# AlexandreGac/alphazero-chess

Measured on AMD Instinct MI355X. Metric: MCTS sims/sec at 800 sims/move, 20x256 net; self-play games/hr at 1/2/4/8 GPU, higher is better.
Workload: dtype f32

## Files before the change

alphazero-chess_amd/azchess/_lib.py:

```python
import ctypes as C
import os

import numpy as np

_HERE = os.path.dirname(os.path.abspath(__file__))
LIB_PATH = os.environ.get("AZ_LIB") or os.path.join(_HERE, "libaz.so")
CSRC = os.path.join(os.path.dirname(_HERE), "csrc")

ACTION_SPACE = 4096
MAX_MOVES = 256
ONGOING, DRAW, WHITE_WINS, BLACK_WINS, ILLEGAL = 0, 1, 2, 3, -1
DTYPE_F32, DTYPE_BF16, DTYPE_FP8 = 0, 1, 2
EVAL_NET, EVAL_SYNTHETIC, EVAL_CALLBACK = 0, 1, 2
PACKED_KINDS = ("conv_w", "conv_b", "in_pk32", "wino_w", "wino16_w", "wino16_us", "w8", "w8s", "b8", "head",
                "head_frag", "head_frag32")


class AzPos(C.Structure):
    _fields_ = [("bb", C.c_uint64 * 8), ("turn", C.c_uint8), ("castling", C.c_uint8), ("ep", C.c_uint8),
                ("flags", C.c_uint8), ("halfmoves", C.c_uint16), ("fullmoves", C.c_uint16),
                ("rep_key", C.c_uint64)]


POS_DTYPE = np.dtype({
# ... 67 lines not shown
    ("az_pos_encode", C.c_int, [P(AzPos), P(C.c_float)]),
    ("az_game_create", C.c_int, [P(C.c_void_p)]),
    ("az_game_clone", C.c_int, [C.c_void_p, P(C.c_void_p)]),
    ("az_game_destroy", C.c_int, [C.c_void_p]),
    ("az_game_position", C.c_int, [C.c_void_p, P(AzPos)]),
    ("az_game_history", C.c_int, [C.c_void_p, P(C.c_int32), C.c_int]),
    ("az_game_play", C.c_int, [C.c_void_p, C.c_int32]),
    ("az_net_num_params", C.c_size_t, [C.c_int, C.c_int]),
    ("az_net_create", C.c_int, [P(AzNetDesc), P(C.c_float), C.c_size_t, C.c_int, P(C.c_void_p)]),
    ("az_net_destroy", C.c_int, [C.c_void_p]),
    ("az_net_tower_kernel", C.c_int, [C.c_void_p, C.c_char_p, C.c_int]),
    ("az_net_wino_streamed_points", C.c_int, [C.c_void_p]),
    ("az_net_wino_accumulators", C.c_int, [C.c_void_p]),
    ("az_net_wino_v_rows", C.c_int, [C.c_void_p]),
    ("az_wino_vrows_layout", C.c_int, [C.c_void_p] * 5),
    ("az_wino16_pack", C.c_int, [P(C.c_float), C.c_int, C.c_int, P(C.c_uint16), C.c_size_t, P(C.c_float)]),
    ("az_wino16_pack_rows", C.c_int, [P(C.c_float), C.c_int, P(C.c_uint16), C.c_size_t, P(C.c_float)]),
    ("az_net_load_mpk",C.c_int, [C.c_char_p, C.c_int, C.c_int, P(C.c_float), C.c_size_t]),
    ("az_net_save_mpk", C.c_int, [C.c_char_p, C.c_int, C.c_int, P(C.c_float), C.c_size_t]),
    ("az_net_forward", C.c_int, [C.c_void_p, P(C.c_float), C.c_int, P(C.c_float), P(C.c_float)]),
    ("az_net_forward_device", C.c_int, [C.c_void_p, C.c_void_p, C.c_int, C.c_void_p, C.c_void_p, C.c_void_p]),
    ("az_net_update_device", C.c_int, [C.c_void_p, C.c_void_p, C.c_size_t, C.c_void_p]),
    ("az_net_update", C.c_int, [C.c_void_p, P(C.c_float), C.c_size_t]),
    ("az_net_update_from_trainer", C.c_int, [C.c_void_p, C.c_void_p]),
    ("az_net_generation", C.c_int64, [C.c_void_p]),
    ("az_net_get_weights", C.c_int, [C.c_void_p, P(C.c_float), C.c_size_t]),
    ("az_net_packed_read", C.c_int, [C.c_void_p, C.c_int, C.c_int, C.c_void_p, C.c_size_t]),
    ("az_search_default_cfg", C.c_int, [P(AzSearchCfg)]),
    ("az_search_create", C.c_int, [C.c_void_p, P(AzSearchCfg), C.c_int, P(C.c_void_p)]),
    ("az_search_destroy", C.c_int, [C.c_void_p]),
# ... 127 lines not shown
```

alphazero-chess_amd/azchess/agent.py:

```python
import ctypes as C
import os

import numpy as np

from . import _lib as L
from .parameters import NUM_FILTERS, NUM_RES_BLOCKS, SEED


def num_params(blocks, filters):
    return int(L.lib.az_net_num_params(int(blocks), int(filters)))


def param_shapes(blocks, filters):
    F = filters
    out = [("input_conv.weight", (F, 19, 3, 3), 19 * 9), ("input_conv.bias", (F,), 19 * 9),
           ("input_bn", (4, F), None)]
    for b in range(blocks):
        for k in (1, 2):
            out += [("res_blocks.%d.conv%d.weight" % (b, k), (F, F, 3, 3), F * 9),
                    ("res_blocks.%d.conv%d.bias" % (b, k), (F,), F * 9),
                    ("res_blocks.%d.bn%d" % (b, k), (4, F), None)]
    out += [("policy_conv_1.weight", (32, F, 1, 1), F), ("policy_conv_1.bias", (32,), F), ("policy_bn", (4, 32), None),
            ("policy_conv_2.weight", (64, 32, 1, 1), 32), ("policy_conv_2.bias", (64,), 32),
            ("value_conv.weight", (8, F, 1, 1), F), ("value_conv.bias", (8,), F), ("value_bn", (4, 8), None),
# ... 95 lines not shown
        return buf.value.decode()

    @property
    def wino_streamed_points(self):
        return L.check(L.lib.az_net_wino_streamed_points(self._h))

    @property
    def wino_accumulators(self):
        return L.check(L.lib.az_net_wino_accumulators(self._h))

    @property
    def wino_v_rows(self):
        return L.check(L.lib.az_net_wino_v_rows(self._h))

    @property
    def winograd(self):
        return "Winograd" in self.tower_kernel

    def __del__(self):
        try:
            L.lib.az_net_destroy(self._h)
        except Exception:
            pass

    def save_file(self, path):
        save_mpk(path, self.weights, self.blocks, self.filters)

    def forward(self, x):
        x = np.ascontiguousarray(x, np.float32).reshape(-1, 19 * 64)
        n = x.shape[0]
        pol = np.zeros((n, 4096), np.float32)
        val = np.zeros(n, np.float32)
        L.check(L.lib.az_net_forward(self._h, L.fptr(x), n, L.fptr(pol), L.fptr(val)))
        return pol, val


def wino_vrows_layout():
    t = dict(write=np.empty((16, 64, 4), np.int32), read=np.empty((2, 4, 4, 64), np.int32),
             act=np.empty((16, 64, 4), np.int32), item=np.empty((2, 8, 4), np.int32), dims=np.empty(4, np.int32))
    L.check(L.lib.az_wino_vrows_layout(*(t[k].ctypes.data_as(C.c_void_p) for k in ("write", "read", "act", "item", "dims"))))
    return t


def mx8_quantize(x):
    x = np.ascontiguousarray(x, np.float32)
    if x.size % 32:
        raise ValueError("mx8_quantize: %d values are not whole blocks of 32" % x.size)
    codes = np.empty(x.shape, np.uint8)
    scales = np.empty(x.size // 32, np.uint8)
    u8 = lambda a: a.ctypes.data_as(L.P(C.c_uint8))
    L.check(L.lib.az_mx8_quantize(L.fptr(x), x.size // 32, u8(codes), u8(scales)))
    return codes, scales


def mx8_conv_probe(filters, act_codes, act_scales, w_codes, w_scales, bias, residual=None, device=0):
# ... 21 lines not shown
```

alphazero-chess_amd/csrc/api.hip:

```cpp
#include <string.h>

#include <cstdio>
#include <string>
#include <vector>

#include "az_internal.h"

namespace azi {
static thread_local std::string g_err;
void set_error(const std::string& m) { g_err = m; }
int fail(const std::string& m) { g_err = m; return -1; }
}

using namespace azi;

namespace {
inline const azc::Pos& P(const az_pos* p) { return *reinterpret_cast<const azc::Pos*>(p); }
inline azc::Pos& P(az_pos* p) { return *reinterpret_cast<azc::Pos*>(p); }

struct VecSink {
    int32_t* out; int cap; int n;
    void operator()(int idx) {
        const int reps = (idx & azc::PROMO_FLAG) ? 4 : 1;
        for (int r = 0; r < reps; r++) { if (n < cap) out[n] = idx & azc::IDX_MASK; n++; }
// ... 256 lines not shown
    return n->fused && tower_supported(n) && wino_split16(n) ? n->wino_streamed : 0;
}

int az_net_wino_accumulators(az_net* net) {
    if (!net) return fail("null argument");
    const NetDev* n = net->dev;
    return n->fused && tower_supported(n) && wino_split16(n) ? (n->wino_rows ? 8 : 16) : 0;
}

int az_net_wino_v_rows(az_net* net) {
    if (!net) return fail("null argument");
    const NetDev* n = net->dev;
    return n->fused && tower_supported(n) && wino_split16(n) && n->wino_rows && n->wino_vrows ? 1 : 0;
}

int az_wino16_pack(const float* folded, int filters, int streamed, uint16_t* out, size_t cap, float* unscale) {
    return wino16_pack(folded, filters, streamed, out, cap, unscale);
}

int az_wino16_pack_rows(const float* folded, int filters, uint16_t* out, size_t cap, float* unscale) {
    return wino16_pack_rows(folded, filters, out, cap, unscale);
}

static int ensure_scratch(NetDev* n, int rows) {
    if (rows <= n->scratch_rows) return 0;
    (void)hipFree(n->x); (void)hipFree(n->h); (void)hipFree(n->planes);
    n->x = n->h = n->planes = nullptr;
    const size_t ab = act_bytes(n->dtype);
    AZ_HIP(hipMalloc(&n->x, (size_t)rows * 64 * n->filters * ab));
    AZ_HIP(hipMalloc(&n->h, (size_t)rows * 64 * n->filters * ab));
// ... 46 lines not shown
```

alphazero-chess_amd/csrc/az_internal.h:

```cpp
#pragma once
#include <hip/hip_runtime.h>
#include <stdint.h>
#include <string>
#include <vector>

#include "../../include/az.h"
#include "chess.h"

static_assert(sizeof(az_pos) == 80, "az_pos layout");
static_assert(sizeof(azc::Pos) == sizeof(az_pos), "Pos == az_pos");

#ifndef AZ_WINOGRAD_DEFAULT
#define AZ_WINOGRAD_DEFAULT 1
#endif
#ifndef AZ_WINO_SPLIT16_DEFAULT
#define AZ_WINO_SPLIT16_DEFAULT 1
#endif
#ifndef AZ_WINO_DERIVE_DEFAULT
#define AZ_WINO_DERIVE_DEFAULT 1
#endif
#ifndef AZ_WINO_ROWS_DEFAULT
#define AZ_WINO_ROWS_DEFAULT 1
#endif
#ifndef AZ_WINO_VROWS_DEFAULT
#define AZ_WINO_VROWS_DEFAULT 1
#endif
#ifndef AZ_WINO_VROWS_SCHED
#define AZ_WINO_VROWS_SCHED 0
#endif
#ifndef AZ_WINO_ROWS_PF
#define AZ_WINO_ROWS_PF 4
#endif

namespace azi {

constexpr float WINO16_SA = 64.0f;
static inline bool wino16_selected(int level, int filters) {
    return filters == 256 ? level >= 1 : (filters == 128 || filters == 64) && level >= 2;
}

static inline int wino16_streamed(bool derive, int filters) { return derive && filters == 256 ? 12 : 16; }
constexpr int WINO_ROWS_PF = AZ_WINO_ROWS_PF;
static_assert(12 % WINO_ROWS_PF == 0 && WINO_ROWS_PF >= 2, "the ring's slots must be compile-time");
static inline bool wino16_rows(bool derive, bool rows, int filters) { return wino16_streamed(derive, filters) == 12 && rows; }
static inline bool wino16_vrows(bool rows_form, bool vrows) { return rows_form && vrows; }

void set_error(const std::string& msg);
int fail(const std::string& msg);

#define AZ_HIP(expr)                                                                        \
    do {                                                                                    \
        hipError_t e_ = (expr);                                                             \
        if (e_ != hipSuccess)                                                               \
            return ::azi::fail(std::string(#expr) + ": " + hipGetErrorString(e_));          \
    } while (0)

__device__ __forceinline__ int load_fresh(const int* p) {
    return __hip_atomic_load(p, __ATOMIC_RELAXED, __HIP_MEMORY_SCOPE_AGENT);
}
__device__ __forceinline__ int vgpr_index(int i) {
// ... 87 lines not shown
    std::vector<float*> conv_b;
    std::vector<size_t> conv_bytes;
    std::vector<void*> wino_w;
    std::vector<size_t> wino_bytes;
    bool winograd = AZ_WINOGRAD_DEFAULT != 0;
    std::vector<void*> wino16_w;
    std::vector<size_t> wino16_bytes;
    std::vector<float> wino16_us;
    int split16 = AZ_WINO_SPLIT16_DEFAULT;
    bool wino_derive = AZ_WINO_DERIVE_DEFAULT != 0;
    int wino_streamed = 16;
    bool wino_rows_env = AZ_WINO_ROWS_DEFAULT != 0;
    bool wino_rows = false;
    bool wino_vrows_env = AZ_WINO_VROWS_DEFAULT != 0;
    bool wino_vrows = false;
    float* head = nullptr;
    void* head_frag = nullptr;
    void* in_pk32 = nullptr;
    size_t in_pk32_bytes = 0;
    void* head_frag32 = nullptr;
    void* w8 = nullptr; void* w8s = nullptr; float* b8 = nullptr;
    size_t w8_bytes = 0, w8s_bytes = 0;
    size_t head_floats = 0;
    hipStream_t stream = nullptr;
    bool fused = true;
    void* x = nullptr; void* h = nullptr; void* planes = nullptr; int scratch_rows = 0;
    float* d_in = nullptr; float* d_pol = nullptr; float* d_val = nullptr; int io_rows = 0;
    int64_t generation = 0;
    struct NetUpdate* upd = nullptr;
};
// ... 61 lines not shown
```

alphazero-chess_amd/csrc/net.hip:

```cpp
#include <math.h>
#include <string.h>

#include <algorithm>
#include <cstdio>
#include <cstdlib>

#include "az_internal.h"

namespace azi {

typedef __attribute__((ext_vector_type(8))) __bf16 bf16x8;
typedef __attribute__((ext_vector_type(4))) float f32x4;
typedef __attribute__((ext_vector_type(4))) __bf16 bf16x4;

template <typename T> struct DTraits;
template <> struct DTraits<__bf16> { static constexpr int CH_SLOT = 8; static constexpr int CHUNK = 32; };
template <> struct DTraits<float> { static constexpr int CH_SLOT = 4; static constexpr int CHUNK = 16; };

template <typename T> __device__ __forceinline__ float to_f(T v) { return (float)v; }

size_t act_bytes(int dtype) { return dtype == AZ_DTYPE_F32 ? 4 : 2; }

double net_tower_flop_per_eval(int B, int F) {
    return 2.0 * 64.0 * (171.0 * F + 18.0 * B * (double)F * F);
// ... 521 lines not shown
    const bool fp8 = d->dtype == AZ_DTYPE_FP8;
    if (fp8 && F != 128 && F != 256) return fail("AZ_DTYPE_FP8: the MX-fp8 tower supports 128 or 256 filters, not " + std::to_string(F));
    if (fp8 && B > 40) return fail("AZ_DTYPE_FP8: at most 40 blocks");
    if (fp8 && getenv("AZ_FUSED_TOWER") && atoi(getenv("AZ_FUSED_TOWER")) == 0)
        return fail("AZ_DTYPE_FP8 has only the fused tower kernel (AZ_FUSED_TOWER=0 is set)");
    if (n != az_net_num_params(B, F)) return fail("weight count mismatch");
    AZ_HIP(hipSetDevice(device));
    NetDev* net = new NetDev();
    net->blocks = B; net->filters = F; net->dtype = d->dtype; net->device = device;
    if (const char* e = getenv("AZ_FUSED_TOWER")) net->fused = atoi(e) != 0;
    if (const char* e = getenv("AZ_WINOGRAD")) net->winograd = atoi(e) != 0;
    if (const char* e = getenv("AZ_WINO_SPLIT16")) net->split16 = atoi(e);
    if (const char* e = getenv("AZ_WINO_DERIVE")) net->wino_derive = atoi(e) != 0;
    if (const char* e = getenv("AZ_WINO_ROWS")) net->wino_rows_env = atoi(e) != 0;
    if (const char* e = getenv("AZ_WINO_VROWS")) net->wino_vrows_env = atoi(e) != 0;
    AZ_HIP(hipStreamCreateWithFlags(&net->stream, hipStreamNonBlocking));
    const float* p = wts;
    std::vector<uint8_t> w8h, w8sh;
    std::vector<float> b8h;
    auto fold_conv = [&](int cin, const float* w, const float* bias, const float* bn) {
        const float *gamma = bn, *beta = bn + F, *mean = bn + 2 * F, *var = bn + 3 * F;
        std::vector<float> wf((size_t)F * cin * 9);
        std::vector<float> bf(F);
        for (int co = 0; co < F; co++) {
            const double sc = (double)gamma[co] / sqrt((double)var[co] + 1e-5);
            for (int k = 0; k < cin * 9; k++) wf[(size_t)co * cin * 9 + k] = (float)(w[(size_t)co * cin * 9 + k] * sc);
            bf[co] = (float)(((double)bias[co] - mean[co]) * sc + beta[co]);
        }
        if (fp8 && cin == F) {
            mx8_append_conv(wf, F, &w8h, &w8sh);
// ... 24 lines not shown
        }
        const bool h16 = d->dtype == AZ_DTYPE_F32 && cin == F && net->winograd && wino16_selected(net->split16, F);
        if (d->dtype == AZ_DTYPE_F32 && F >= 64 && cin == F && !h16) {
            auto u = winograd_f32(wf, F);
            void* du = nullptr;
            if (hipMalloc(&du, u.size() * 4) != hipSuccess) return -1;
            if (hipMemcpy(du, u.data(), u.size() * 4, hipMemcpyHostToDevice) != hipSuccess) return -1;
            net->wino_w.push_back(du);
            net->wino_bytes.push_back(u.size() * 4);
        }
        if (h16) {
            float us = 1.0f;
            net->wino_streamed = wino16_streamed(net->wino_derive, F);
            net->wino_rows = wino16_rows(net->wino_derive, net->wino_rows_env, F);
            net->wino_vrows = wino16_vrows(net->wino_rows, net->wino_vrows_env);
            auto u = net->wino_rows ? winograd_split16_rows(wf.data(), F, &us)
                                    : winograd_split16(wf.data(), F, net->wino_streamed, &us);
            void* du = nullptr;
            if (hipMalloc(&du, u.size() * 2) != hipSuccess) return -1;
            if (hipMemcpy(du, u.data(), u.size() * 2, hipMemcpyHostToDevice) != hipSuccess) return -1;
            net->wino16_w.push_back(du);
            net->wino16_bytes.push_back(u.size() * 2);
            net->wino16_us.push_back(us);
        }
        if (hipMalloc(&db, F * 4) != hipSuccess) return -1;
        if (hipMemcpy(db, bf.data(), F * 4, hipMemcpyHostToDevice) != hipSuccess) return -1;
        net->conv_w.push_back(dw);
        net->conv_b.push_back(db);
        return 0;
    };
// ... 81 lines not shown
}

void net_destroy(NetDev* n) {
    if (!n) return;
    (void)hipSetDevice(n->device);
    for (void* w : n->conv_w) (void)hipFree(w);
    for (void* w : n->wino_w) (void)hipFree(w);
    for (void* w : n->wino16_w) (void)hipFree(w);
    for (float* b : n->conv_b) (void)hipFree(b);
    (void)hipFree(n->head);
    (void)hipFree(n->head_frag);
    (void)hipFree(n->head_frag32);
    (void)hipFree(n->in_pk32);
    (void)hipFree(n->w8); (void)hipFree(n->w8s); (void)hipFree(n->b8);
    (void)hipFree(n->x); (void)hipFree(n->h); (void)hipFree(n->planes);
    (void)hipFree(n->d_in); (void)hipFree(n->d_pol); (void)hipFree(n->d_val);
    net_update_free(n);
    if (n->stream) (void)hipStreamDestroy(n->stream);
    delete n;
}

int net_tower(NetDev* n, const void* planes, const int* count, int rows, void* x, void* h, hipStream_t st,
              hipEvent_t ev0, hipEvent_t ev1) {
    if (rows <= 0) return 0;
    const int F = n->filters;
    const bool bf = n->dtype == AZ_DTYPE_BF16;
    int rc = bf ? launch_conv<__bf16>(F, 32, false, planes, x, n->conv_w[0], n->conv_b[0], count, rows, st)
                : launch_conv<float>(F, 32, false, planes, x, n->conv_w[0], n->conv_b[0], count, rows, st);
    if (rc) return rc;
    for (int b = 0; b < n->blocks; b++) {
// ... 96 lines not shown
```

alphazero-chess_amd/csrc/tower.hip:

```cpp
#include <math.h>
#include <stdio.h>
#include <stdlib.h>
#include <string.h>

#include "az_internal.h"
#include "search_dev.h"
#include "wino.h"

#include "tower_dev.h"

namespace azi {

template <int F, bool SEARCH>
__device__ __forceinline__ void tower_board(const __bf16* __restrict__ planes, const TowerArgs& ta, int row0, int nb,
                                            float* __restrict__ pol_out, float* __restrict__ val_out,
                                            const SearchOut& so, int tid) {
    constexpr int BPB = TowerCfg<F>::BPB, WB = TowerCfg<F>::WB, BPW = BPB / WB, NCO = TowerCfg<F>::NCO;
    constexpr int NCW = F / (16 * NCO);
    constexpr int NT = NCW * WB * 64;
    constexpr int RSF = F / 8 + 2, RSI = 32 / 8 + 2;
    constexpr int XSZ = BPB * 64 * RSF;
    constexpr int ZN = 16 + F / 8;
    constexpr int HSZ0 = (HeadsScratch<HeadsCfg<F>::NB, NT>::FLOATS * 4 + 15) / 16;
    constexpr int HSZ = ((XSZ > HSZ0 ? XSZ : HSZ0) + 15) / 16 * 16;
// ... 505 lines not shown
    }
    heads_group<F, RSF, 1, NT, SEARCH, true, H16>(ldsb, reinterpret_cast<float*>(V), 0, 1, row0, tid, ta.head_frag32, ta.head,
                                             pol_out, val_out, so, tr);
    wino_stamp(tr, 3 + 64 * 20);
}

template <int F, bool SEARCH, bool H16, int SP = 16, bool ROWS = false, bool VROWS = false>
__global__ void __launch_bounds__(WinoCfg<F>::NWV * 64)
tower32w_kernel(const float* __restrict__ planes, TowerArgs ta, const int* __restrict__ count_ptr, int rows,
                float* __restrict__ pol_out, float* __restrict__ val_out, SearchOut so) {
    const int count = count_ptr ? min(load_fresh(count_ptr), rows) : rows;
    if ((int)blockIdx.x >= count) return;
    tower32w_board<F, SEARCH, H16, SP, ROWS, VROWS>(planes, ta, blockIdx.x, pol_out, val_out, so, threadIdx.x);
}

template <int F, bool BF16> struct SimsCfg { static constexpr int NT = WinoCfg<F>::NWV * 64; };
template <int F> struct SimsCfg<F, true> {
    static_assert(TowerCfg<F>::BPB == 1, "persistent bf16 kernel: one board per workgroup");
    static constexpr int NT = (F / (16 * TowerCfg<F>::NCO)) * TowerCfg<F>::WB * 64;
};
template <int F, bool BF16, bool H16 = false, int SP = 16, bool ROWS = false, bool VROWS = false>
__global__ void __launch_bounds__((SimsCfg<F, BF16>::NT))
k_sims32w(Engine E, TowerArgs ta, SearchOut so, int step0, int step1) {
    __shared__ int s_kind;
    if (!E.active[vgpr_index(blockIdx.x)]) return;
    for (int step = step0; step <= step1; step++) {
        const int tid = vgpr_index(threadIdx.x), g = vgpr_index(blockIdx.x);
        const int lane = tid & 63, w = __builtin_amdgcn_readfirstlane(tid >> 6);
        unsigned long long* tr = tt_slot(w);
        wino_stamp(tr, 1910);
// ... 93 lines not shown
    if (n->filters == FF) {                                                                            \
        k_sims32w<FF, false, H16, SP, ROWS, VR><<<E.G, SimsCfg<FF, false>::NT, 0, st>>>(E, ta, so, step0, step1); \
        return hipGetLastError() == hipSuccess ? 0 : fail("persistent simulation kernel launch failed"); \
    }
    if (wino_split16(n)) {
        if (n->wino_streamed == 12 && n->wino_rows && n->wino_vrows) { AZ_SIMS32W(256, true, 12, true, true) }
        if (n->wino_streamed == 12 && n->wino_rows) { AZ_SIMS32W(256, true, 12, true, false) }
        if (n->wino_streamed == 12) { AZ_SIMS32W(256, true, 12, false, false) }
        AZ_SIMS32W(256, true, 16, false, false) AZ_SIMS32W(128, true, 16, false, false) AZ_SIMS32W(64, true, 16, false, false)
    }
    AZ_SIMS32W(256, false, 16, false, false) AZ_SIMS32W(128, false, 16, false, false) AZ_SIMS32W(64, false, 16, false, false)
#undef AZ_SIMS32W
    return fail("persistent simulation kernel: unsupported filters");
}

int tower_forward(NetDev* n, const void* planes, const int* count, int rows, float* pol, float* val,
                  const SearchOut* so, hipStream_t st) {
    if (rows <= 0) return 0;
    if (!tower_supported(n)) return fail("fused tower: unsupported net");
    if (!planes && (!so || !so->npos)) return fail("fused tower: no planes and no leaf positions to encode");
    if (n->dtype == AZ_DTYPE_FP8) return tower8_forward(n, planes, count, rows, pol, val, so, st);
    TowerArgs ta = tower_args(n);
    SearchOut dummy;
    memset(&dummy, 0, sizeof(dummy));
    const SearchOut& s = so ? *so : dummy;
#define AZ_TOWER(FF)                                                                                           \
    if (n->filters == FF) {                                                                                    \
        constexpr int BPB = TowerCfg<FF>::BPB;                                                                 \
        constexpr int NT = (FF / (16 * TowerCfg<FF>::NCO)) * TowerCfg<FF>::WB * 64;                            \
        const int grid = (rows + BPB - 1) / BPB;                                                               \
// ... 7 lines not shown
        constexpr int NT = (FF / (16 * Tower32Cfg<FF>::NCO)) * Tower32Cfg<FF>::WB * 64;                        \
        const int grid = (rows + BPB - 1) / BPB;                                                               \
        if (so) tower32_kernel<FF, true><<<grid, NT, 0, st>>>((const float*)planes, ta, count, rows, pol, val, s); \
        else tower32_kernel<FF, false><<<grid, NT, 0, st>>>((const float*)planes, ta, count, rows, pol, val, s);  \
        return hipGetLastError() == hipSuccess ? 0 : fail("f32 tower launch failed");                          \
    }
    if (n->dtype == AZ_DTYPE_F32) {
#define AZ_TOWER32W(FF, H16, SP, ROWS, VR)                                                                       \
        if (n->filters == FF) {                                                                                \
            constexpr int NT = WinoCfg<FF>::NWV * 64;                                                          \
            if (so) tower32w_kernel<FF, true, H16, SP, ROWS, VR><<<rows, NT, 0, st>>>((const float*)planes, ta, count, rows, pol, val, s); \
            else tower32w_kernel<FF, false, H16, SP, ROWS, VR><<<rows, NT, 0, st>>>((const float*)planes, ta, count, rows, pol, val, s);  \
            return hipGetLastError() == hipSuccess ? 0 : fail("f32 Winograd tower launch failed");             \
        }
        if (wino_split16(n)) {
            if (n->wino_streamed == 12 && n->wino_rows && n->wino_vrows) { AZ_TOWER32W(256, true, 12, true, true) }
            if (n->wino_streamed == 12 && n->wino_rows) { AZ_TOWER32W(256, true, 12, true, false) }
            if (n->wino_streamed == 12) { AZ_TOWER32W(256, true, 12, false, false) }
            AZ_TOWER32W(256, true, 16, false, false) AZ_TOWER32W(128, true, 16, false, false) AZ_TOWER32W(64, true, 16, false, false)
        }
        if (wino_supported(n)) {
            AZ_TOWER32W(256, false, 16, false, false) AZ_TOWER32W(128, false, 16, false, false) AZ_TOWER32W(64, false, 16, false, false)
        }
#undef AZ_TOWER32W
        AZ_TOWER32(256) AZ_TOWER32(128) AZ_TOWER32(64) AZ_TOWER32(32)
        return fail("fused tower: unsupported filters");
    }
    AZ_TOWER(256) AZ_TOWER(128) AZ_TOWER(64) AZ_TOWER(32)
#undef AZ_TOWER
#undef AZ_TOWER32
// ... 15 lines not shown
        for (int b = 0; b < 4; b++)
            for (int lane = 0; lane < 64; lane++) {
                read[(i * 4 + b) * 64 + lane] = wino_vr_read(i, b, lane);
                read[((4 + i) * 4 + b) * 64 + lane] = wino_vr_lo(wino_vr_rlane(lane, i >> 1)) + wino_vr_rimm(i, b);
            }
    for (int sched = 0; sched < 2; sched++)
        for (int wave = 0; wave < 8; wave++)
            for (int it = 0; it < 4; it++) {
                const int nw = sched ? 8 : 4;
                item[(sched * 8 + wave) * 4 + it] = wave < nw && it < WINO_VR_ITEMS / nw ? wino_vr_item(wave, it, nw) : -1;
            }
    dims[0] = WINO_VR_PLANE; dims[1] = WINO_VR_BYTES; dims[2] = WINO_VR_R16; dims[3] = 4;
    return 0;
}

#ifdef AZ_TOWER_TRACE
extern "C" int az_tower_trace_read(unsigned long long* out, size_t n) {
    const size_t cap = sizeof(azi::az_tower_trace_buf) / sizeof(unsigned long long);
    if (hipDeviceSynchronize() != hipSuccess) return -1;
    return hipMemcpyFromSymbol(out, HIP_SYMBOL(azi::az_tower_trace_buf), (n < cap ? n : cap) * 8) == hipSuccess ? 0 : -1;
}
#endif
```

alphazero-chess_amd/csrc/wino.h:

```cpp
#pragma once
#include "az_internal.h"

namespace azi {

typedef __attribute__((ext_vector_type(4))) float f32x4;
typedef __attribute__((ext_vector_type(2))) float f32x2;

#define AZ_PK2(name, mods)                                                                    \
    __device__ __forceinline__ f32x2 name(f32x2 a, f32x2 b) {                                 \
        f32x2 r;                                                                              \
        asm("v_pk_add_f32 %0, %1, %2 " mods : "=v"(r) : "v"(a), "v"(b));                      \
        return r;                                                                             \
    }
#define AZ_PK3(name, mods)                                                                    \
    __device__ __forceinline__ f32x2 name(f32x2 a, f32x2 m, f32x2 b) {                        \
        f32x2 r;                                                                              \
        asm("v_pk_fma_f32 %0, %1, %2, %3 " mods : "=v"(r) : "v"(a), "v"(m), "v"(b));          \
        return r;                                                                             \
    }
AZ_PK2(pk_add, "")
AZ_PK2(pk_sub, "neg_lo:[0,1] neg_hi:[0,1]")
AZ_PK2(pk_rowa, "op_sel_hi:[1,0] neg_lo:[0,1]")
AZ_PK2(pk_rowb, "op_sel:[1,0] neg_lo:[0,1] neg_hi:[0,1]")
AZ_PK2(pk_negx_add, "neg_lo:[1,1]")
// ... 716 lines not shown
                    s1[j] = pk_sub(pk_sub(m[4 + j], m[8 + j]), m[12 + j]);
                }
            }
            const f32x2 q0 = pkc_fma(pk_add(pk_add(s0[0], s0[1]), s0[2]), us, br);
            const f32x2 q1 = pkc_fma(pk_sub(pk_sub(s0[1], s0[2]), s0[3]), us, br);
            const f32x2 q2 = pkc_fma(pk_add(pk_add(s1[0], s1[1]), s1[2]), us, br);
            const f32x2 q3 = pkc_fma(pk_sub(pk_sub(s1[1], s1[2]), s1[3]), us, br);
            y[n][0][2 * p] = q0.x; y[n][0][2 * p + 1] = q0.y;
            y[n][1][2 * p] = q1.x; y[n][1][2 * p + 1] = q1.y;
            y[n][2][2 * p] = q2.x; y[n][2][2 * p + 1] = q2.y;
            y[n][3][2 * p] = q3.x; y[n][3][2 * p + 1] = q3.y;
        }
    }
}

}
```

include/az.h:

```cpp
#ifndef AZ_H
#define AZ_H
#include <stddef.h>
#include <stdint.h>

#ifdef __cplusplus
extern "C" {
#endif

#define AZ_ACTION_SPACE 4096
#define AZ_PLANES 19
#define AZ_MAX_MOVES 256

enum { AZ_ONGOING = 0, AZ_DRAW = 1, AZ_WHITE_WINS = 2, AZ_BLACK_WINS = 3, AZ_ILLEGAL = -1 };

typedef struct az_pos {
    uint64_t bb[8];
    uint8_t turn, castling, ep, flags;
    uint16_t halfmoves, fullmoves;
    uint64_t rep_key;
} az_pos;

const char* az_last_error(void);
int az_version(void);
int az_device_count(int* n);
// ... 15 lines not shown
int az_game_destroy(az_game* g);
int az_game_position(const az_game* g, az_pos* out);
int az_game_history(const az_game* g, int32_t* moves, int cap);
int az_game_play(az_game* g, int32_t index);

enum { AZ_DTYPE_F32 = 0, AZ_DTYPE_BF16 = 1, AZ_DTYPE_FP8 = 2 };
typedef struct { int blocks, filters, dtype; } az_net_desc;
typedef struct az_net az_net;
size_t az_net_num_params(int blocks, int filters);
int az_net_create(const az_net_desc* desc, const float* weights, size_t n, int device, az_net** out);
int az_net_destroy(az_net* net);
int az_net_tower_kernel(az_net* net, char* out, int cap);
int az_net_wino_streamed_points(az_net* net);
int az_net_wino_accumulators(az_net* net);
int az_net_wino_v_rows(az_net* net);
int az_wino_vrows_layout(int* write, int* read, int* act, int* item, int* dims);
int az_net_load_mpk(const char* path, int blocks, int filters, float* out, size_t n);
int az_net_save_mpk(const char* path, int blocks, int filters, const float* w, size_t n);
int az_net_forward(az_net* net, const float* planes, int n, float* policy, float* value);
int az_net_forward_device(az_net* net, const float* d_planes, int n, float* d_policy, float* d_value,
                          void* stream);
int az_net_update_device(az_net* net, const float* d_weights, size_t n, void* stream);
int az_net_update(az_net* net, const float* weights, size_t n);
int64_t az_net_generation(az_net* net);
int az_net_get_weights(az_net* net, float* out, size_t n);
enum {
    AZ_PACKED_CONV_W = 0, AZ_PACKED_CONV_B = 1, AZ_PACKED_IN_PK32 = 2, AZ_PACKED_WINO_W = 3, AZ_PACKED_WINO16_W = 4,
    AZ_PACKED_WINO16_US = 5, AZ_PACKED_W8 = 6, AZ_PACKED_W8S = 7, AZ_PACKED_B8 = 8, AZ_PACKED_HEAD = 9,
    AZ_PACKED_HEAD_FRAG = 10, AZ_PACKED_HEAD_FRAG32 = 11, AZ_PACKED_KINDS = 12
};
// ... 167 lines not shown
```

Measured before the change: 191,600.

## Add two-board-per-workgroup Winograd tower kernel with global activation buffers

Adds a new fused tower kernel where each 512-thread workgroup runs two boards through the 20-block Winograd tower. Every weight fragment loaded from memory then feeds MFMAs for both boards, which halves weight traffic per board. Activations move from LDS to a per-stream global scratch buffer, leaving LDS room for two boards' transformed tiles. Waves coordinate through an LDS flag. It is on by default for 256-filter f32 split16 rows/vrows nets. The cost is extra global-memory round-trips for activations and more register pressure.

```diff
diff --git a/alphazero-chess_amd/azchess/_lib.py b/alphazero-chess_amd/azchess/_lib.py
--- a/alphazero-chess_amd/azchess/_lib.py
+++ b/alphazero-chess_amd/azchess/_lib.py
@@ -105,6 +105,8 @@
     ("az_net_wino_accumulators", C.c_int, [C.c_void_p]),
     ("az_net_wino_v_rows", C.c_int, [C.c_void_p]),
     ("az_wino_vrows_layout", C.c_int, [C.c_void_p] * 5),
+    ("az_net_wino_boards", C.c_int, [C.c_void_p]),
+    ("az_wino_boards_layout", C.c_int, [C.c_void_p] * 6),
     ("az_wino16_pack", C.c_int, [P(C.c_float), C.c_int, C.c_int, P(C.c_uint16), C.c_size_t, P(C.c_float)]),
     ("az_wino16_pack_rows", C.c_int, [P(C.c_float), C.c_int, P(C.c_uint16), C.c_size_t, P(C.c_float)]),
     ("az_net_load_mpk",C.c_int, [C.c_char_p, C.c_int, C.c_int, P(C.c_float), C.c_size_t]),
diff --git a/alphazero-chess_amd/azchess/agent.py b/alphazero-chess_amd/azchess/agent.py
--- a/alphazero-chess_amd/azchess/agent.py
+++ b/alphazero-chess_amd/azchess/agent.py
@@ -133,6 +133,10 @@
         return L.check(L.lib.az_net_wino_v_rows(self._h))
 
     @property
+    def wino_boards(self):
+        return L.check(L.lib.az_net_wino_boards(self._h))
+
+    @property
     def winograd(self):
         return "Winograd" in self.tower_kernel
 
@@ -158,6 +162,13 @@
     t = dict(write=np.empty((16, 64, 4), np.int32), read=np.empty((2, 4, 4, 64), np.int32),
              act=np.empty((16, 64, 4), np.int32), item=np.empty((2, 8, 4), np.int32), dims=np.empty(4, np.int32))
     L.check(L.lib.az_wino_vrows_layout(*(t[k].ctypes.data_as(C.c_void_p) for k in ("write", "read", "act", "item", "dims"))))
+    return t
+
+
+def wino_boards_layout():
+    t = dict(item=np.empty((8, 8, 2), np.int32), act=np.empty((2, 2), np.int32), out=np.empty((8, 64, 2, 4), np.int32),
+             vbuf=np.empty((2, 2), np.int32), zero=np.empty(64, np.int32), dims=np.empty(8, np.int32))
+    L.check(L.lib.az_wino_boards_layout(*(t[k].ctypes.data_as(C.c_void_p) for k in ("item", "act", "out", "vbuf", "zero", "dims"))))
     return t
 
 
diff --git a/alphazero-chess_amd/csrc/api.hip b/alphazero-chess_amd/csrc/api.hip
--- a/alphazero-chess_amd/csrc/api.hip
+++ b/alphazero-chess_amd/csrc/api.hip
@@ -294,6 +294,13 @@
     return n->fused && tower_supported(n) && wino_split16(n) && n->wino_rows && n->wino_vrows ? 1 : 0;
 }
 
+int az_net_wino_boards(az_net* net) {
+    if (!net) return fail("null argument");
+    const NetDev* n = net->dev;
+    if (!(n->fused && tower_supported(n) && wino_split16(n))) return 0;
+    return n->wino_rows && n->wino_vrows ? n->wino_boards : 1;
+}
+
 int az_wino16_pack(const float* folded, int filters, int streamed, uint16_t* out, size_t cap, float* unscale) {
     return wino16_pack(folded, filters, streamed, out, cap, unscale);
 }
diff --git a/alphazero-chess_amd/csrc/az_internal.h b/alphazero-chess_amd/csrc/az_internal.h
--- a/alphazero-chess_amd/csrc/az_internal.h
+++ b/alphazero-chess_amd/csrc/az_internal.h
@@ -1,6 +1,8 @@
 #pragma once
 #include <hip/hip_runtime.h>
 #include <stdint.h>
+#include <map>
+#include <mutex>
 #include <string>
 #include <vector>
 
@@ -27,6 +29,9 @@
 #endif
 #ifndef AZ_WINO_VROWS_SCHED
 #define AZ_WINO_VROWS_SCHED 0
+#endif
+#ifndef AZ_WINO_BOARDS_DEFAULT
+#define AZ_WINO_BOARDS_DEFAULT 2
 #endif
 #ifndef AZ_WINO_ROWS_PF
 #define AZ_WINO_ROWS_PF 4
@@ -44,6 +49,7 @@
 static_assert(12 % WINO_ROWS_PF == 0 && WINO_ROWS_PF >= 2, "the ring's slots must be compile-time");
 static inline bool wino16_rows(bool derive, bool rows, int filters) { return wino16_streamed(derive, filters) == 12 && rows; }
 static inline bool wino16_vrows(bool rows_form, bool vrows) { return rows_form && vrows; }
+static inline int wino16_boards(bool vrows_form, int boards) { return vrows_form && boards == 2 ? 2 : 1; }
 
 void set_error(const std::string& msg);
 int fail(const std::string& msg);
@@ -161,6 +167,11 @@
     bool wino_rows = false;
     bool wino_vrows_env = AZ_WINO_VROWS_DEFAULT != 0;
     bool wino_vrows = false;
+    int wino_boards_env = AZ_WINO_BOARDS_DEFAULT;
+    int wino_boards = 1;
+    struct B2Act { void* p = nullptr; int wgs = 0; };
+    std::map<hipStream_t, B2Act> b2_act;
+    std::mutex b2_mu;
     float* head = nullptr;
     void* head_frag = nullptr;
     void* in_pk32 = nullptr;
diff --git a/alphazero-chess_amd/csrc/net.hip b/alphazero-chess_amd/csrc/net.hip
--- a/alphazero-chess_amd/csrc/net.hip
+++ b/alphazero-chess_amd/csrc/net.hip
@@ -559,6 +559,7 @@
     if (const char* e = getenv("AZ_WINO_DERIVE")) net->wino_derive = atoi(e) != 0;
     if (const char* e = getenv("AZ_WINO_ROWS")) net->wino_rows_env = atoi(e) != 0;
     if (const char* e = getenv("AZ_WINO_VROWS")) net->wino_vrows_env = atoi(e) != 0;
+    if (const char* e = getenv("AZ_WINO_BOARDS")) net->wino_boards_env = atoi(e);
     AZ_HIP(hipStreamCreateWithFlags(&net->stream, hipStreamNonBlocking));
     const float* p = wts;
     std::vector<uint8_t> w8h, w8sh;
@@ -613,6 +614,7 @@
             net->wino_streamed = wino16_streamed(net->wino_derive, F);
             net->wino_rows = wino16_rows(net->wino_derive, net->wino_rows_env, F);
             net->wino_vrows = wino16_vrows(net->wino_rows, net->wino_vrows_env);
+            net->wino_boards = wino16_boards(net->wino_vrows, net->wino_boards_env);
             auto u = net->wino_rows ? winograd_split16_rows(wf.data(), F, &us)
                                     : winograd_split16(wf.data(), F, net->wino_streamed, &us);
             void* du = nullptr;
@@ -724,6 +726,7 @@
     (void)hipFree(n->in_pk32);
     (void)hipFree(n->w8); (void)hipFree(n->w8s); (void)hipFree(n->b8);
     (void)hipFree(n->x); (void)hipFree(n->h); (void)hipFree(n->planes);
+    for (auto& kv : n->b2_act) (void)hipFree(kv.second.p);
     (void)hipFree(n->d_in); (void)hipFree(n->d_pol); (void)hipFree(n->d_val);
     net_update_free(n);
     if (n->stream) (void)hipStreamDestroy(n->stream);
diff --git a/alphazero-chess_amd/csrc/tower.hip b/alphazero-chess_amd/csrc/tower.hip
--- a/alphazero-chess_amd/csrc/tower.hip
+++ b/alphazero-chess_amd/csrc/tower.hip
@@ -543,6 +543,177 @@
     tower32w_board<F, SEARCH, H16, SP, ROWS, VROWS>(planes, ta, blockIdx.x, pol_out, val_out, so, threadIdx.x);
 }
 
+typedef unsigned int u32v4 __attribute__((__vector_size__(16)));
+constexpr int WINO_B2_HS = (HeadsScratch<1, 512, heads_npart(512, true)>::FLOATS * 4 + 15) / 16;
+constexpr int WINO_B2_AUX = ((WINO_B2_HS > 64 * 10 ? WINO_B2_HS : 64 * 10) + 15) / 16 * 16;
+constexpr int WINO_B2_ZN = 16 + 256 / 4;
+constexpr int WINO_B2_LDS = (WINO_B2_VBYTES / 16 + WINO_B2_AUX + WINO_B2_ZN + 1) * 16;
+constexpr int WINO_B2_OVL = 0;
+static_assert(WINO_B2_OVL % 256 == 0 && WINO_B2_OVL + WINO_B2_ACT <= WINO_B2_VBYTES, "the ACT overlay lies inside V");
+__device__ __forceinline__ void b2_stores_done() { asm volatile("s_waitcnt vmcnt(0)" ::: "memory"); }
+
+template <bool RESID>
+__device__ __forceinline__ void conv_wino_b2(char* __restrict__ ldsv, const __amdgpu_buffer_rsrc_t rW,
+                                             const __amdgpu_buffer_rsrc_t rN, const __amdgpu_buffer_rsrc_t rA,
+                                             const float* __restrict__ bias, float unscale,
+                                             f32x4 (&wr)[WINO_B2_PF][2][2], int w, int lane, bool pre_in, bool pre_out,
+                                             int* flag, int seq, unsigned long long* tr = nullptr) {
+    constexpr int HIN = RESID ? 1 : 0, HOUT = 1 - HIN;
+    f32x4 acc[2][8][2];
+    wino_stamp(tr, 0);
+    wino_core_b2(ldsv, rW, rN, rA, HIN, wr, w, lane, pre_in, acc, tr);
+    wino_stamp(tr, 10);
+    const int ln = vgpr_index(lane);
+    const int co0 = w * 32 + (ln >> 4) * 4;
+    auto out_addr = [&](int n, int a, int b) { return wino_b2_out(w, ln, n, 2 * a + b); };
+    f32x4 xres[2][4];
+    auto xload = [&](int k) {
+        if constexpr (RESID) {
+#pragma unroll
+            for (int q = 0; q < 4; q++)
+                xres[k & 1][q] = __builtin_bit_cast(f32x4, __builtin_amdgcn_raw_buffer_load_b128(
+                                                               rA, wino_b2_act(k >> 1, 0) + out_addr(k & 1, q >> 1, q & 1), 0, 0));
+        }
+    };
+    xload(0);
+    xload(1);
+    (void)xres;
+#pragma unroll
+    for (int nb = 0; nb < 2; nb++)
+#pragma unroll
+        for (int n = 0; n < 2; n++) {
+            f32x4 y[4];
+            wino_rows_out(acc[nb], bias, unscale, co0, n, y);
+            f32x4 o[4];
+#pragma unroll
+            for (int q = 0; q < 4; q++) {
+                o[q] = y[q];
+                if constexpr (RESID) o[q] += xres[n][q];
+            }
+            if (2 * nb + n + 2 < 4) xload(2 * nb + n + 2);
+#pragma unroll
+            for (int q = 0; q < 4; q++) {
+                f32x4 v = o[q];
+#pragma unroll
+                for (int r = 0; r < 4; r++) v[r] = relu_nan<true>(v[r]);
+                __builtin_amdgcn_raw_buffer_store_b128(__builtin_bit_cast(u32v4, v), rA,
+                                                       wino_b2_act(nb, HOUT) + out_addr(n, q >> 1, q & 1), 0, 0);
+            }
+        }
+    wino_stamp(tr, 11);
+    b2_stores_done();
+    if (pre_out && w < 4) {
+        if (w == 0) __hip_atomic_store(flag, seq, __ATOMIC_RELEASE, __HIP_MEMORY_SCOPE_WORKGROUP);
+        else
+            while (__hip_atomic_load(flag, __ATOMIC_ACQUIRE, __HIP_MEMORY_SCOPE_WORKGROUP) != seq)
+                __builtin_amdgcn_s_sleep(1);
+        wino_b2_items<4>(ldsv, rA, HOUT, 0, 0, w, lane);
+    }
+    __syncthreads();
+}
+
+template <bool SEARCH>
+__device__ __forceinline__ void tower32w_boards2(const float* __restrict__ planes, const TowerArgs& ta, int row0, int nbv,
+                                                 char* __restrict__ act, float* __restrict__ pol_out,
+                                                 float* __restrict__ val_out, const SearchOut& so, int tid) {
+    constexpr int F = 256, NT = 512, NN = 2, RSF = F / 4 + 2, RSI = 32 / 4 + 2, PF = WINO_B2_PF;
+    constexpr int VSZ = WINO_B2_VBYTES / 16, AUX = WINO_B2_AUX, ZN = WINO_B2_ZN;
+    static_assert(64 * RSF <= VSZ && 64 * RSF * 16 == WINO_B2_ACT, "one board's ACT overlays V");
+    static_assert(64 * RSI <= AUX, "input planes must fit in AUX");
+    static_assert((VSZ + AUX) * 16 % 256 == 0, "conv32_in_packed ORs the zero row's offset into the low byte");
+    static_assert(WINO_B2_LDS <= 163840, "LDS of a CU");
+    __shared__ __attribute__((aligned(16))) uint4 lds[VSZ + AUX + ZN + 1];
+    const int lane = tid & 63;
+    const int w = __builtin_amdgcn_readfirstlane(tid >> 6);
+    char* ldsb = reinterpret_cast<char*>(lds);
+    char* actl = ldsb + WINO_B2_OVL;
+    uint4* A = lds + VSZ;
+    const int zero_off = (VSZ + AUX) * 16;
+    int* flag = reinterpret_cast<int*>(lds + VSZ + AUX + ZN);
+    const __amdgpu_buffer_rsrc_t rA = t32_rsrc(reinterpret_cast<const uint4*>(act), WINO_B2_WG);
+    unsigned long long* tr = nullptr;
+#ifdef AZ_TOWER_TRACE
+    tr = tt_slot(w);
+#endif
+    wino_stamp(tr, 0);
+    for (int c = tid; c < ZN + 1; c += NT) lds[VSZ + AUX + c] = make_uint4(0, 0, 0, 0);
+#pragma unroll 1
+    for (int nb = 0; nb < 2; nb++) {
+        stage_planes_f32<1, RSI, NT>(A, planes, so, row0 + nb, nb < nbv ? 1 : 0, tid);
+        __syncthreads();
+        if (nb == 0) wino_stamp(tr, 1);
+        {
+            f32x4 wr[T32_PF][NN];
+            const __amdgpu_buffer_rsrc_t r0 = t32_rsrc(ta.w0pk, ta.w0pk_bytes);
+            const int voff = ((w * NN) * 64 + lane) * 16;
+#pragma unroll
+            for (int i = 0; i < T32_PF; i++)
+#pragma unroll
+                for (int n = 0; n < NN; n++)
+                    wr[i][n] = __builtin_bit_cast(f32x4, __builtin_amdgcn_raw_buffer_load_b128(
+                                                             r0, voff + n * 1024 + i * (F / 16) * 1024, 0, 0));
+            conv32_in_packed<F, RSI, RSF, NN>(ldsb, actl, VSZ * 16, zero_off, r0, ta.b[0], wr, w, lane);
+        }
+        for (int i = tid; i < 64 * 64; i += NT) {
+            const int o = ((i >> 6) * RSF + (i & 63)) * 16;
+            __builtin_amdgcn_raw_buffer_store_b128(*reinterpret_cast<const u32v4*>(actl + o), rA, wino_b2_act(nb, 0) + o, 0, 0);
+        }
+        b2_stores_done();
+        __syncthreads();
+    }
+    static_assert(NT == 32 * 16, "two uint4 of the zero rows per thread");
+#pragma unroll
+    for (int k = 0; k < 2; k++)
+        *reinterpret_cast<uint4*>(ldsb + wino_vr_zero((tid >> 4) + 32 * k) + (tid & 15) * 16) = make_uint4(0, 0, 0, 0);
+    wino_stamp(tr, 2);
+    f32x4 wring[PF][2][NN];
+    if (ta.blocks > 0) {
+        const __amdgpu_buffer_rsrc_t r = t32_rsrc(ta.ww[0], ta.wwbytes[0]);
+        const int voff = wino16_voff<F>(w, lane);
+#pragma unroll
+        for (int i = 0; i < PF; i++)
+#pragma unroll
+            for (int pl = 0; pl < 2; pl++)
+#pragma unroll
+                for (int n = 0; n < NN; n++)
+                    wring[i][pl][n] = __builtin_bit_cast(f32x4, __builtin_amdgcn_raw_buffer_load_b128(
+                                                                    r, voff + (2 * n + pl) * 1024 + i * (F / 16) * 2048, 0, 0));
+    }
+    for (int b = 0; b < ta.blocks; b++) {
+        const unsigned wb3 = b + 1 < ta.blocks ? ta.wwbytes[2 * b + 2] : 0u;
+        const __amdgpu_buffer_rsrc_t r1 = t32_rsrc(ta.ww[2 * b], ta.wwbytes[2 * b]);
+        const __amdgpu_buffer_rsrc_t r2 = t32_rsrc(ta.ww[2 * b + 1], ta.wwbytes[2 * b + 1]);
+        const __amdgpu_buffer_rsrc_t r3 = t32_rsrc(b + 1 < ta.blocks ? ta.ww[2 * b + 2] : ta.ww[2 * b + 1], wb3);
+        conv_wino_b2<false>(ldsb, r1, r2, rA, ta.b[1 + 2 * b], ta.wus[2 * b], wring, w, lane, b > 0, true, flag, 2 * b + 1,
+                            tr ? tr + 3 + 64 * b : nullptr);
+        conv_wino_b2<true>(ldsb, r2, r3, rA, ta.b[2 + 2 * b], ta.wus[2 * b + 1], wring, w, lane, true, b + 1 < ta.blocks, flag,
+                           2 * b + 2, tr ? tr + 35 + 64 * b : nullptr);
+    }
+    tid = w * 64 + (int)__builtin_amdgcn_mbcnt_hi(~0u, __builtin_amdgcn_mbcnt_lo(~0u, 0u));
+#pragma unroll 1
+    for (int nb = 0; nb < nbv; nb++) {
+        for (int i = tid; i < 64 * 64; i += NT) {
+            const int o = ((i >> 6) * RSF + (i & 63)) * 16;
+            *reinterpret_cast<u32v4*>(actl + o) = __builtin_amdgcn_raw_buffer_load_b128(rA, wino_b2_act(nb, 0) + o, 0, 0);
+        }
+        __syncthreads();
+        heads_group<F, RSF, 1, NT, SEARCH, true, true>(actl, reinterpret_cast<float*>(A), 0, 1, row0 + nb, tid, ta.head_frag32,
+                                                       ta.head, pol_out, val_out, so, tr);
+    }
+    wino_stamp(tr, 3 + 64 * 20);
+}
+
+template <bool SEARCH>
+__global__ void __launch_bounds__(512)
+tower32w2_kernel(const float* __restrict__ planes, TowerArgs ta, const int* __restrict__ count_ptr, int rows,
+                 char* __restrict__ act, float* __restrict__ pol_out, float* __restrict__ val_out, SearchOut so) {
+    const int count = count_ptr ? min(load_fresh(count_ptr), rows) : rows;
+    const int row0 = 2 * (int)blockIdx.x;
+    if (row0 >= count) return;
+    tower32w_boards2<SEARCH>(planes, ta, row0, min(2, count - row0), act + (size_t)blockIdx.x * WINO_B2_WG, pol_out, val_out,
+                             so, threadIdx.x);
+}
+
 template <int F, bool BF16> struct SimsCfg { static constexpr int NT = WinoCfg<F>::NWV * 64; };
 template <int F> struct SimsCfg<F, true> {
     static_assert(TowerCfg<F>::BPB == 1, "persistent bf16 kernel: one board per workgroup");
@@ -666,6 +837,21 @@
     return fail("persistent simulation kernel: unsupported filters");
 }
 
+static char* b2_act_for(NetDev* n, hipStream_t st, int wgs) {
+    std::lock_guard<std::mutex> lock(n->b2_mu);
+    NetDev::B2Act& a = n->b2_act[st];
+    if (wgs > a.wgs) {
+        if (a.p) {
+            if (hipStreamSynchronize(st) != hipSuccess) return nullptr;
+            (void)hipFree(a.p);
+        }
+        a = NetDev::B2Act();
+        if (hipMalloc(&a.p, (size_t)wgs * WINO_B2_WG) != hipSuccess) { a.p = nullptr; return nullptr; }
+        a.wgs = wgs;
+    }
+    return static_cast<char*>(a.p);
+}
+
 int tower_forward(NetDev* n, const void* planes, const int* count, int rows, float* pol, float* val,
                   const SearchOut* so, hipStream_t st) {
     if (rows <= 0) return 0;
@@ -703,6 +889,14 @@
             return hipGetLastError() == hipSuccess ? 0 : fail("f32 Winograd tower launch failed");             \
         }
         if (wino_split16(n)) {
+            if (n->filters == 256 && n->wino_streamed == 12 && n->wino_rows && n->wino_vrows && n->wino_boards == 2) {
+                const int grid = (rows + 1) / 2;
+                char* act = b2_act_for(n, st, grid);
+                if (!act) return fail("two-board tower: global activations allocation failed");
+                if (so) tower32w2_kernel<true><<<grid, 512, 0, st>>>((const float*)planes, ta, count, rows, act, pol, val, s);
+                else tower32w2_kernel<false><<<grid, 512, 0, st>>>((const float*)planes, ta, count, rows, act, pol, val, s);
+                return hipGetLastError() == hipSuccess ? 0 : fail("f32 Winograd tower launch failed");
+            }
             if (n->wino_streamed == 12 && n->wino_rows && n->wino_vrows) { AZ_TOWER32W(256, true, 12, true, true) }
             if (n->wino_streamed == 12 && n->wino_rows) { AZ_TOWER32W(256, true, 12, true, false) }
             if (n->wino_streamed == 12) { AZ_TOWER32W(256, true, 12, false, false) }
@@ -748,6 +942,29 @@
     return 0;
 }
 
+extern "C" int az_wino_boards_layout(int* item, int* act, int* out, int* vbuf, int* zero, int* dims) {
+    using namespace azi;
+    if (!item || !act || !out || !vbuf || !zero || !dims) return fail("null argument");
+    for (int w = 0; w < 8; w++)
+        for (int k = 0; k < 8; k++) {
+            item[(w * 8 + k) * 2] = k < wino_b2_item_count(w) ? wino_b2_item_board(w, k) : -1;
+            item[(w * 8 + k) * 2 + 1] = k < wino_b2_item_count(w) ? wino_b2_item_q(w, k) : -1;
+        }
+    for (int nb = 0; nb < 2; nb++)
+        for (int b = 0; b < 2; b++) {
+            act[nb * 2 + b] = wino_b2_act(nb, b);
+            vbuf[nb * 2 + b] = wino_b2_v(nb, b);
+        }
+    for (int w = 0; w < 8; w++)
+        for (int lane = 0; lane < 64; lane++)
+            for (int n = 0; n < 2; n++)
+                for (int q = 0; q < 4; q++) out[((w * 64 + lane) * 2 + n) * 4 + q] = wino_b2_out(w, lane, n, q);
+    for (int k = 0; k < 64; k++) zero[k] = wino_vr_zero(k);
+    dims[0] = WINO_B2_ACT; dims[1] = WINO_B2_WG; dims[2] = WINO_VR_BYTES; dims[3] = WINO_B2_OVL; dims[4] = WINO_B2_ACT;
+    dims[5] = WINO_B2_VBYTES; dims[6] = WINO_B2_AUX * 16; dims[7] = WINO_B2_LDS;
+    return 0;
+}
+
 #ifdef AZ_TOWER_TRACE
 extern "C" int az_tower_trace_read(unsigned long long* out, size_t n) {
     const size_t cap = sizeof(azi::az_tower_trace_buf) / sizeof(unsigned long long);
diff --git a/alphazero-chess_amd/csrc/wino.h b/alphazero-chess_amd/csrc/wino.h
--- a/alphazero-chess_amd/csrc/wino.h
+++ b/alphazero-chess_amd/csrc/wino.h
@@ -754,4 +754,168 @@
     }
 }
 
-}
+constexpr int WINO_B2_ACT = 64 * WINO_VR_R16;
+constexpr int WINO_B2_BOARD = 2 * WINO_B2_ACT;
+constexpr int WINO_B2_WG = 2 * WINO_B2_BOARD;
+constexpr int WINO_B2_VBYTES = 4 * WINO_VR_BYTES;
+#ifndef AZ_WINO_B2_PF
+#define AZ_WINO_B2_PF 3
+#endif
+constexpr int WINO_B2_PF = AZ_WINO_B2_PF;
+static_assert(12 % WINO_B2_PF == 0 && WINO_B2_PF >= 2, "the ring's slots must be compile-time");
+__host__ __device__ constexpr int wino_b2_act(int nb, int hbuf) { return nb * WINO_B2_BOARD + hbuf * WINO_B2_ACT; }
+__host__ __device__ constexpr int wino_b2_v(int nb, int buf) { return (2 * nb + buf) * WINO_VR_BYTES; }
+__host__ __device__ constexpr int wino_b2_out(int w, int lane, int n, int q) {
+    const int l16 = lane & 15, ty = l16 >> 2, tx = l16 & 3;
+    return ((2 * ty + (q >> 1)) * 8 + 2 * tx + (q & 1)) * WINO_VR_R16 + (w * 32 + (lane >> 4) * 4 + n * 16) * 4;
+}
+#ifndef AZ_WINO_B2_XE
+#define AZ_WINO_B2_XE 6
+#endif
+constexpr int WINO_B2_XE = AZ_WINO_B2_XE, WINO_B2_XL = 8 - WINO_B2_XE;
+static_assert(WINO_B2_XE >= 4 && WINO_B2_XE <= 8, "waves 0-3 take at least their share, at most everything");
+__host__ __device__ constexpr int wino_b2_item_count(int w) { return w < 4 ? WINO_B2_XE : WINO_B2_XL; }
+__host__ __device__ constexpr int wino_b2_item_g(int w, int k) { return w < 4 ? w + 4 * k : 4 * WINO_B2_XE + (w - 4) + 4 * k; }
+__host__ __device__ constexpr int wino_b2_item_board(int w, int k) { return wino_b2_item_g(w, k) >> 4; }
+__host__ __device__ constexpr int wino_b2_item_q(int w, int k) { return wino_b2_item_g(w, k) & 15; }
+
+__device__ __forceinline__ void wino_b2_load(const __amdgpu_buffer_rsrc_t rA, int aoff, int c, int q, float (&e)[4], int ln) {
+    const int tl = ln >> 4;
+    const int p = wino_vr_alane(ln) + wino_vr_auni(q) + c * 128 + aoff;
+#pragma unroll
+    for (int j = 0; j < 4; j++)
+        e[j] = __builtin_bit_cast(float, __builtin_amdgcn_raw_buffer_load_b32(rA, p + wino_vr_acol(tl, j), 0, 0));
+}
+template <int NW>
+__device__ __forceinline__ void wino_b2_items(char* __restrict__ ldsv, const __amdgpu_buffer_rsrc_t rA, int hbuf, int c,
+                                              int buf, int w, int lane) {
+    constexpr int NI = WINO_VR_ITEMS / NW;
+    const int ln = vgpr_index(lane);
+    float e[2][NI][4];
+#pragma unroll
+    for (int nb = 0; nb < 2; nb++)
+#pragma unroll
+        for (int i = 0; i < NI; i++) wino_b2_load(rA, wino_b2_act(nb, hbuf), c, wino_vr_item(w, i, NW), e[nb][i], ln);
+#pragma unroll
+    for (int nb = 0; nb < 2; nb++) {
+        const WinoXf<256> xf(ldsv, wino_b2_v(nb, 0), w, lane);
+#pragma unroll
+        for (int i = 0; i < NI; i++) xf.vr_store(buf, wino_vr_item(w, i, NW), e[nb][i], ln);
+    }
+}
+
+__device__ __forceinline__ void wino_rows_out(const f32x4 (&acc)[8][2], const float* __restrict__ bias, float unscale,
+                                              int co0, int n, f32x4 (&y)[4]) {
+    const f32x2 us = f32x2{unscale, unscale};
+    {
+        const f32x4 bb = *reinterpret_cast<const f32x4*>(bias + co0 + n * 16);
+#pragma unroll
+        for (int p = 0; p < 2; p++) {
+            f32x2 s0[4], s1[4];
+#pragma unroll
+            for (int j = 0; j < 4; j++) {
+                s0[j] = p ? f32x2{acc[j][n][2], acc[j][n][3]} : f32x2{acc[j][n][0], acc[j][n][1]};
+                s1[j] = p ? f32x2{acc[4 + j][n][2], acc[4 + j][n][3]} : f32x2{acc[4 + j][n][0], acc[4 + j][n][1]};
+            }
+            const f32x2 br = p ? f32x2{bb[2], bb[3]} : f32x2{bb[0], bb[1]};
+            const f32x2 q0 = pkc_fma(pk_add(pk_add(s0[0], s0[1]), s0[2]), us, br);
+            const f32x2 q1 = pkc_fma(pk_sub(pk_sub(s0[1], s0[2]), s0[3]), us, br);
+            const f32x2 q2 = pkc_fma(pk_add(pk_add(s1[0], s1[1]), s1[2]), us, br);
+            const f32x2 q3 = pkc_fma(pk_sub(pk_sub(s1[1], s1[2]), s1[3]), us, br);
+            y[0][2 * p] = q0.x; y[0][2 * p + 1] = q0.y;
+            y[1][2 * p] = q1.x; y[1][2 * p + 1] = q1.y;
+            y[2][2 * p] = q2.x; y[2][2 * p + 1] = q2.y;
+            y[3][2 * p] = q3.x; y[3][2 * p + 1] = q3.y;
+        }
+    }
+}
+
+__device__ __forceinline__ void wino_core_b2(char* __restrict__ ldsv, const __amdgpu_buffer_rsrc_t rW,
+                                             const __amdgpu_buffer_rsrc_t rN, const __amdgpu_buffer_rsrc_t rA, int hin,
+                                             f32x4 (&wr)[WINO_B2_PF][2][2], int w, int lane, bool pre,
+                                             f32x4 (&acc)[2][8][2], unsigned long long* tr = nullptr) {
+    constexpr int F = 256, CF = F / 16, NN = 2, PF = WINO_B2_PF, NCHUNK = 8, SPX = 12, STEPB = CF * 2 * 1024;
+    const int vr0 = wino_vr_rlane(lane, 0), vr1 = wino_vr_rlane(lane, 1);
+#pragma unroll
+    for (int nb = 0; nb < 2; nb++)
+#pragma unroll
+        for (int x = 0; x < 8; x++)
+#pragma unroll
+            for (int n = 0; n < NN; n++) {
+                f32x2 z0, z1;
+                asm volatile("v_mov_b64 %0, 0" : "=v"(z0));
+                asm volatile("v_mov_b64 %0, 0" : "=v"(z1));
+                acc[nb][x][n] = f32x4{z0.x, z0.y, z1.x, z1.y};
+            }
+    const int voff = wino16_voff<F>(w, lane);
+    if (!pre) {
+        wino_b2_items<8>(ldsv, rA, hin, 0, 0, w, lane);
+        __syncthreads();
+    }
+    wino_stamp(tr, 1);
+#pragma unroll 1
+    for (int c = 0; c < NCHUNK; c++) {
+        const bool more = c + 1 < NCHUNK;
+        f16x8 bw[2][2][2];
+        float en[4];
+        auto bread = [&](int nb, int st) {
+            const char* vb = ldsv + wino_b2_v(nb, c & 1);
+#pragma unroll
+            for (int s = st % 3 == 0 ? 0 : 1; s < 2; s++) {
+                const int n = 4 * (st / 3) + st % 3 + s;
+                const int vl = (n % 4) >> 1 ? vr1 : vr0;
+                const char* p = vb + wino_vr_rimm(n % 4, n / 4);
+                bw[nb][n % 2][0] = *reinterpret_cast<const f16x8*>(p + vl);
+                bw[nb][n % 2][1] = *reinterpret_cast<const f16x8*>(p + wino_vr_lo(vl));
+            }
+        };
+        bread(0, 0);
+        bread(1, 0);
+#pragma unroll
+        for (int st = 0; st < SPX; st++) {
+            const int b = st / 3;
+            if (more) {
+                if (st >= 1 && st <= wino_b2_item_count(w)) {
+                    const WinoXf<F> xf(ldsv, wino_b2_v(wino_b2_item_board(w, st - 1), 0), w, lane);
+                    xf.vr_store((c + 1) & 1, wino_b2_item_q(w, st - 1), en, vgpr_index(lane));
+                }
+                if (st < wino_b2_item_count(w))
+                    wino_b2_load(rA, wino_b2_act(wino_b2_item_board(w, st), hin), c + 1, wino_b2_item_q(w, st), en, vgpr_index(lane));
+            }
+#pragma unroll
+            for (int nb = 0; nb < 2; nb++) {
+                __builtin_amdgcn_sched_barrier(0);
+#pragma unroll
+                for (int term = 0; term < 3; term++)
+#pragma unroll
+                    for (int pt = 0; pt < 2; pt++)
+#pragma unroll
+                        for (int n = 0; n < NN; n++) {
+                            const f16x8 av = __builtin_bit_cast(f16x8, wr[st % PF][term == 2 ? 1 : 0][n]);
+                            const f16x8 bv = bw[nb][(4 * b + st % 3 + pt) % 2][term == 1 ? 1 : 0];
+                            acc[nb][4 * pt + b][n] = __builtin_amdgcn_mfma_f32_16x16x32_f16(av, bv, acc[nb][4 * pt + b][n], 0, 0, 0);
+                        }
+                __builtin_amdgcn_sched_barrier(0);
+                if (nb == 1) {
+                    const bool nxt = st + PF >= SPX && !more;
+                    const int tn = c * SPX + st + PF;
+                    const int to = nxt ? tn - NCHUNK * SPX : tn;
+#pragma unroll
+                    for (int pl = 0; pl < 2; pl++)
+#pragma unroll
+                        for (int n = 0; n < NN; n++)
+                            wr[st % PF][pl][n] = __builtin_bit_cast(
+                                f32x4, __builtin_amdgcn_raw_buffer_load_b128(nxt ? rN : rW, voff + (2 * n + pl) * 1024,
+                                                                             to * STEPB, 0));
+                }
+                if (st + 1 < SPX) bread(nb, st + 1);
+            }
+            if (st == 4) wino_stamp(tr, 20 + c);
+        }
+        wino_stamp(tr, 12 + c);
+        if (more) __syncthreads();
+        wino_stamp(tr, 2 + c);
+    }
+}
+
+}
diff --git a/include/az.h b/include/az.h
--- a/include/az.h
+++ b/include/az.h
@@ -53,6 +53,8 @@
 int az_net_wino_streamed_points(az_net* net);
 int az_net_wino_accumulators(az_net* net);
 int az_net_wino_v_rows(az_net* net);
+int az_net_wino_boards(az_net* net);
+int az_wino_boards_layout(int* item, int* act, int* out, int* vbuf, int* zero, int* dims);
 int az_wino_vrows_layout(int* write, int* read, int* act, int* item, int* dims);
 int az_net_load_mpk(const char* path, int blocks, int filters, float* out, size_t n);
 int az_net_save_mpk(const char* path, int blocks, int filters, const float* w, size_t n);
```

Result: faster. 209,900 (median of 6 runs) (+9.5%).
